# louislung/DAE_RNN_News_Recommendation

Measured on NVIDIA H100. Metric: articles/sec, higher is better.
Workload: dtype f32

## Files before the change

dae_rnn_news_recommendation_b200/csrc/gemm_tc.cu:

```cuda
#include <cuda.h>
#include <cuda_bf16.h>
#include <type_traits>
#include "common.cuh"

namespace dae {

constexpr int BLOCK_M = 128;
constexpr int BLOCK_K = 64;
constexpr int WGMMA_K = 16;
constexpr int kThreads = 384;
constexpr int kDecodeN = 128;

__device__ __forceinline__ uint32_t smem_u32(const void* p) { return (uint32_t)__cvta_generic_to_shared(p); }

__device__ __forceinline__ void mbar_init(uint64_t* bar, uint32_t count) {
  asm volatile("mbarrier.init.shared::cta.b64 [%0], %1;" ::"r"(smem_u32(bar)), "r"(count));
}
__device__ __forceinline__ void mbar_expect_tx(uint64_t* bar, uint32_t bytes) {
  asm volatile("mbarrier.arrive.expect_tx.shared::cta.b64 _, [%0], %1;" ::"r"(smem_u32(bar)), "r"(bytes) : "memory");
}
__device__ __forceinline__ void mbar_arrive(uint64_t* bar) {
  asm volatile("mbarrier.arrive.shared::cta.b64 _, [%0];" ::"r"(smem_u32(bar)) : "memory");
}
__device__ __forceinline__ bool mbar_try_wait(uint64_t* bar, uint32_t parity) {
// ... 79 lines not shown
  d |= (uint64_t)layout << 62;
  return d;
}


template <int TA, int TB>
__device__ __forceinline__ void wgmma_n128(float (&d)[64], uint64_t da, uint64_t db, uint32_t scale_d) {
  asm volatile(
      "{\n"
      ".reg .pred p;\n"
      "setp.ne.b32 p, %66, 0;\n"
      "wgmma.mma_async.sync.aligned.m64n128k16.f32.bf16.bf16 "
      "{%0, %1, %2, %3, %4, %5, %6, %7, %8, %9, %10, %11, %12, %13, %14, %15, %16, %17, %18, %19, %20, %21, %22, %23, %24, %25, %26, %27, %28, %29, %30, %31, %32, %33, %34, %35, %36, %37, %38, %39, %40, %41, %42, %43, %44, %45, %46, %47, %48, %49, %50, %51, %52, %53, %54, %55, %56, %57, %58, %59, %60, %61, %62, %63}, %64, %65, p, 1, 1, %67, %68;\n"
      "}\n"
      : "+f"(d[0]), "+f"(d[1]), "+f"(d[2]), "+f"(d[3]), "+f"(d[4]), "+f"(d[5]), "+f"(d[6]), "+f"(d[7]), "+f"(d[8]), "+f"(d[9]), "+f"(d[10]), "+f"(d[11]), "+f"(d[12]), "+f"(d[13]), "+f"(d[14]), "+f"(d[15]), "+f"(d[16]), "+f"(d[17]), "+f"(d[18]), "+f"(d[19]), "+f"(d[20]), "+f"(d[21]), "+f"(d[22]), "+f"(d[23]), "+f"(d[24]), "+f"(d[25]), "+f"(d[26]), "+f"(d[27]), "+f"(d[28]), "+f"(d[29]), "+f"(d[30]), "+f"(d[31]), "+f"(d[32]), "+f"(d[33]), "+f"(d[34]), "+f"(d[35]), "+f"(d[36]), "+f"(d[37]), "+f"(d[38]), "+f"(d[39]), "+f"(d[40]), "+f"(d[41]), "+f"(d[42]), "+f"(d[43]), "+f"(d[44]), "+f"(d[45]), "+f"(d[46]), "+f"(d[47]), "+f"(d[48]), "+f"(d[49]), "+f"(d[50]), "+f"(d[51]), "+f"(d[52]), "+f"(d[53]), "+f"(d[54]), "+f"(d[55]), "+f"(d[56]), "+f"(d[57]), "+f"(d[58]), "+f"(d[59]), "+f"(d[60]), "+f"(d[61]), "+f"(d[62]), "+f"(d[63])
      : "l"(da), "l"(db), "r"(scale_d), "n"(TA), "n"(TB));
}

template <int TA, int TB>
__device__ __forceinline__ void wgmma_n64(float (&d)[32], uint64_t da, uint64_t db, uint32_t scale_d) {
  asm volatile(
      "{\n"
      ".reg .pred p;\n"
      "setp.ne.b32 p, %34, 0;\n"
      "wgmma.mma_async.sync.aligned.m64n64k16.f32.bf16.bf16 "
      "{%0, %1, %2, %3, %4, %5, %6, %7, %8, %9, %10, %11, %12, %13, %14, %15, %16, %17, %18, %19, %20, %21, %22, %23, %24, %25, %26, %27, %28, %29, %30, %31}, %32, %33, p, 1, 1, %35, %36;\n"
      "}\n"
      : "+f"(d[0]), "+f"(d[1]), "+f"(d[2]), "+f"(d[3]), "+f"(d[4]), "+f"(d[5]), "+f"(d[6]), "+f"(d[7]), "+f"(d[8]), "+f"(d[9]), "+f"(d[10]), "+f"(d[11]), "+f"(d[12]), "+f"(d[13]), "+f"(d[14]), "+f"(d[15]), "+f"(d[16]), "+f"(d[17]), "+f"(d[18]), "+f"(d[19]), "+f"(d[20]), "+f"(d[21]), "+f"(d[22]), "+f"(d[23]), "+f"(d[24]), "+f"(d[25]), "+f"(d[26]), "+f"(d[27]), "+f"(d[28]), "+f"(d[29]), "+f"(d[30]), "+f"(d[31])
      : "l"(da), "l"(db), "r"(scale_d), "n"(TA), "n"(TB));
}
// ... 7 lines not shown
  int a_sym_kb;
  float alpha;
  float* C;
  int64_t ldc;
  int n_store;
  int special_col;
  float* special_out;
  const int64_t* indptr; const int32_t* indices; const float* values; const int32_t* rows;
  const float* bv; const float* weight; const double* stats;
  __nv_bfloat16* dz_hi; __nv_bfloat16* dz_lo; int64_t ld_dz;
  float* row_loss_part;
  const int32_t* tile_ptr;
};

struct Sched {
  int tiles_m, tiles, kb_total, kb_per_split, n_work, stream, w, n_cta;
  long long u, u_end;
  __device__ __forceinline__ void init(const GemmParams& p, int block_n, int pair = 0, int block_k = BLOCK_K) {
    const int cta = pair ? (int)(blockIdx.x >> 1) : (int)blockIdx.x;
    n_cta = pair ? (int)(gridDim.x >> 1) : (int)gridDim.x;
    tiles_m = (p.M + BLOCK_M - 1) / BLOCK_M;
    if (pair) tiles_m = (tiles_m + 1) / 2;
    tiles = tiles_m * ((p.N + block_n - 1) / block_n);
    kb_total = (p.K + block_k - 1) / block_k;
    stream = p.stream_k;
    kb_per_split = (kb_total + p.k_splits - 1) / p.k_splits;
    n_work = tiles * p.k_splits;
    w = cta;
    const long long U = (long long)tiles * kb_total;
    u = (long long)cta * U / n_cta;
    u_end = (long long)(cta + 1) * U / n_cta;
  }
  __device__ __forceinline__ bool next(int& mb, int& nb, int& kb0, int& kb1) {
    int tile;
    if (stream) {
      if (u >= u_end) return false;
      tile = (int)(u / kb_total);
      kb0 = (int)(u - (long long)tile * kb_total);
      const long long left = u_end - u;
      kb1 = (left < (long long)(kb_total - kb0)) ? kb0 + (int)left : kb_total;
      u += kb1 - kb0;
    } else {
      if (w >= n_work) return false;
      tile = w % tiles;
      kb0 = (w / tiles) * kb_per_split;
      kb1 = min(kb_total, kb0 + kb_per_split);
      w += n_cta;
    }
    mb = tile % tiles_m;
    nb = tile / tiles_m;
    return true;
  }
};

__device__ __forceinline__ uint32_t pack_bf16(float a, float b) {
  const __nv_bfloat162 v = __floats2bfloat162_rn(a, b);
  return *reinterpret_cast<const uint32_t*>(&v);
}
__device__ __forceinline__ float f_rcp(float x) { float r; asm("rcp.approx.ftz.f32 %0, %1;" : "=f"(r) : "f"(x)); return r; }
__device__ __forceinline__ float f_lg2(float x) { float r; asm("lg2.approx.ftz.f32 %0, %1;" : "=f"(r) : "f"(x)); return r; }
__device__ __forceinline__ float f_ex2(float x) { float r; asm("ex2.approx.ftz.f32 %0, %1;" : "=f"(r) : "f"(x)); return r; }
constexpr float kLog2e = 1.4426950408889634f;

template <int ACT>
__device__ __forceinline__ float act_fast(float z) {
// ... 54 lines not shown
    }
    const float p01 = a[0] * a[1], p23 = a[2] * a[3], P = p01 * p23;
    ok = ok && (P <= 22026.0f);
    const float Rs = f_rcp(P) * sc;
    lsum += f_lg2(P);
    const float r23 = Rs * p23, r01 = Rs * p01;
    const float dz0 = t[0] * (r23 * a[1]), dz1 = t[1] * (r23 * a[0]), dz2 = t[2] * (r01 * a[3]), dz3 = t[3] * (r01 * a[2]);
    const uint32_t h0 = pack_bf16(dz0, dz1), h1 = pack_bf16(dz2, dz3);
    hpk[2 * g] = h0; hpk[2 * g + 1] = h1;
    lpk[2 * g] = pack_bf16(dz0 - __uint_as_float(h0 << 16), dz1 - __uint_as_float(h0 & 0xffff0000u));
    lpk[2 * g + 1] = pack_bf16(dz2 - __uint_as_float(h1 << 16), dz3 - __uint_as_float(h1 & 0xffff0000u));
  }
  return ok;
}

template <int BLOCK_N, int TA, int TB, int BK = BLOCK_K>
__device__ __forceinline__ void mma_kblock(float (&acc)[BLOCK_N / 2], uint32_t sa_hi, uint32_t sa_lo, uint32_t sb_hi, uint32_t sb_lo,
                                           bool first) {
  static_assert(BK == 64 || (BK == 32 && !TA && !TB), "32-wide k-blocks are K-major only");
  constexpr uint32_t layout = BK == 64 ? 1u : 2u, sbo = BK == 64 ? 1024u : 512u;
  constexpr uint32_t a_lbo = TA ? 8192u : 16u, b_lbo = TB ? 8192u : 16u;
  constexpr uint32_t a_step = TA ? 2048u : 32u, b_step = TB ? 2048u : 32u;
#pragma unroll
  for (int k = 0; k < BK / WGMMA_K; ++k) {
    const uint64_t da_hi = make_desc(sa_hi + k * a_step, a_lbo, sbo, layout), da_lo = make_desc(sa_lo + k * a_step, a_lbo, sbo, layout);
    const uint64_t db_hi = make_desc(sb_hi + k * b_step, b_lbo, sbo, layout), db_lo = make_desc(sb_lo + k * b_step, b_lbo, sbo, layout);
    const uint32_t sc = (first && k == 0) ? 0u : 1u;
    if constexpr (BLOCK_N == 128) {
      wgmma_n128<TA, TB>(acc, da_lo, db_hi, sc);
      wgmma_n128<TA, TB>(acc, da_hi, db_lo, 1u);
      wgmma_n128<TA, TB>(acc, da_hi, db_hi, 1u);
    } else {
      wgmma_n64<TA, TB>(acc, da_lo, db_hi, sc);
      wgmma_n64<TA, TB>(acc, da_hi, db_lo, 1u);
      wgmma_n64<TA, TB>(acc, da_hi, db_hi, 1u);
    }
  }
}

__device__ __forceinline__ void stage_ld16(const float* src, uint32_t (&r)[16]) {
#pragma unroll
  for (int q = 0; q < 4; ++q) {
    const float4 v = reinterpret_cast<const float4*>(src)[q];
// ... 50 lines not shown
      } else if (!p.b_mn) {
        tma_load_2d(tm_b_hi, &full_bar[stage], sb_hi, kbb * BK, nb * BLOCK_N);
        tma_load_2d(tm_b_lo, &full_bar[stage], sb_lo, kbb * BK, nb * BLOCK_N);
      } else {
#pragma unroll
        for (int j = 0; j < BLOCK_N / 64; ++j) {
          tma_load_2d(tm_b_hi, &full_bar[stage], sb_hi + j * (64 * BK * 2), nb * BLOCK_N + j * 64, kbb * BK);
          tma_load_2d(tm_b_lo, &full_bar[stage], sb_lo + j * (64 * BK * 2), nb * BLOCK_N + j * 64, kbb * BK);
        }
      }
      if (++stage == STAGES) { stage = 0; phase ^= 1; }
    }
  }
}

template <int BLOCK_N, int STAGES, int PAIR, int MAJ, int BK = BLOCK_K>
__device__ __forceinline__ void mma_work_item(float (&acc)[BLOCK_N / 2], const GemmParams& p, uint8_t* smem, uint64_t* full_bar,
                                              uint64_t* empty_bar, int wg, int lane, uint32_t crank, int& stage, uint32_t& phase,
                                              int kb0, int kb1) {
  constexpr int A_TILE = BLOCK_M * BK * 2;
  constexpr int B_TILE = BLOCK_N * BK * 2;
  constexpr int STAGE_BYTES = 2 * A_TILE + 2 * B_TILE;
  auto release = [&](int s) {
    __syncwarp();
    if (lane == 0) { mbar_arrive(&empty_bar[s]); if (PAIR) mbar_arrive_cluster(&empty_bar[s], crank ^ 1u); }
  };
  int prev = -1;
  auto run_k = [&](auto ta, auto tb, int kb_begin, int kb_end) {
    for (int kb = kb_begin; kb < kb_end; ++kb) {
      mbar_wait(&full_bar[stage], phase);
      const uint32_t sa_hi = smem_u32(smem + stage * STAGE_BYTES) + wg * (64 * BK * 2);
      const uint32_t sa_lo = sa_hi + A_TILE;
      const uint32_t sb_hi = smem_u32(smem + stage * STAGE_BYTES) + 2 * A_TILE, sb_lo = sb_hi + B_TILE;
      wgmma_fence();
      mma_kblock<BLOCK_N, decltype(ta)::value, decltype(tb)::value, BK>(acc, sa_hi, sa_lo, sb_hi, sb_lo, kb == kb0);
      wgmma_commit();
      wgmma_wait<1>();
      if (prev >= 0) release(prev);
      prev = stage;
      if (++stage == STAGES) { stage = 0; phase ^= 1; }
    }
  };
  using K0 = std::integral_constant<int, 0>;
  using K1 = std::integral_constant<int, 1>;
  if constexpr ((MAJ & 4) != 0) {
    run_k(K0{}, K1{}, kb0, min(kb1, p.a_sym_kb));
    run_k(K1{}, K1{}, max(kb0, p.a_sym_kb), kb1);
  } else {
    run_k(std::integral_constant<int, MAJ & 1>{}, std::integral_constant<int, (MAJ >> 1) & 1>{}, kb0, kb1);
  }
// ... 95 lines not shown
                float* dst = p.C + (int64_t)mm * p.ldc + n;
                if (p.atomic) atomicAdd(dst, v); else *dst = v;
              }
            }
          }
        }
      }
    }
  }

  if (PAIR) cluster_sync_all();
}

constexpr int kDecodeThreads = 640;
constexpr int kDecodeBK = 32;
constexpr int kDecodeStages = 4;
constexpr int kRegsProducer = 32, kRegsMma = 104, kRegsEpilogue = 120;
static_assert(128 * kRegsProducer + 256 * kRegsMma + 256 * kRegsEpilogue <= kDecodeThreads * 96, "register budget");

template <int R> __device__ __forceinline__ void regs_dec() { asm volatile("setmaxnreg.dec.sync.aligned.u32 %0;" ::"n"(R)); }
template <int R> __device__ __forceinline__ void regs_inc() { asm volatile("setmaxnreg.inc.sync.aligned.u32 %0;" ::"n"(R)); }

template <int ACT, int LOSS>
__global__ void __launch_bounds__(kDecodeThreads, 1) decode_fused_kernel(const __grid_constant__ CUtensorMap tm_a_hi,
                                                                         const __grid_constant__ CUtensorMap tm_a_lo,
                                                                         const __grid_constant__ CUtensorMap tm_b_hi,
                                                                         const __grid_constant__ CUtensorMap tm_b_lo,
                                                                         const GemmParams p) {
  constexpr int BLOCK_N = kDecodeN, STAGES = kDecodeStages, BK = kDecodeBK;
  constexpr int STAGE_BYTES = 2 * BLOCK_M * BK * 2 + 2 * BLOCK_N * BK * 2;
  constexpr int SROW = BLOCK_N + 4;
  constexpr int kParts = 2;
  constexpr int HALF_N = BLOCK_N / kParts;
  constexpr bool kFast = (ACT == DAE_ACT_SIGMOID) && (LOSS == DAE_LOSS_CE);
  extern __shared__ __align__(1024) uint8_t smem_raw[];
  uint8_t* smem = reinterpret_cast<uint8_t*>((reinterpret_cast<uintptr_t>(smem_raw) + 1023) & ~(uintptr_t)1023);
  float* stg = reinterpret_cast<float*>(smem + STAGES * STAGE_BYTES);
  __shared__ __align__(8) uint64_t full_bar[STAGES], empty_bar[STAGES], staged_bar[2], drained_bar[2];
  __shared__ float s_bias[2][BLOCK_N];
  __shared__ float s_biasc[kFast ? 2 : 1][kFast ? BLOCK_N : 1];
  __shared__ __align__(16) uint8_t s_stage[8][2][32][48];

  const int warp = threadIdx.x >> 5, lane = threadIdx.x & 31;
  const int role = warp >> 2;
  Sched sched;

  if (warp == 0 && lane == 0) { prefetch_tmap(&tm_a_hi); prefetch_tmap(&tm_a_lo); prefetch_tmap(&tm_b_hi); prefetch_tmap(&tm_b_lo); }
  if (warp == 1 && lane == 0) {
    for (int s = 0; s < STAGES; ++s) { mbar_init(&full_bar[s], 1); mbar_init(&empty_bar[s], 8); }
    for (int h = 0; h < 2; ++h) { mbar_init(&staged_bar[h], 4); mbar_init(&drained_bar[h], 4); }
    fence_barrier_init();
  }
  __syncthreads();

  if (role == 0) {
    regs_dec<kRegsProducer>();
    sched.init(p, BLOCK_N, 0, BK);
    if (warp == 0 && lane == 0)
      tma_produce<BLOCK_N, STAGES, 0, BK>(p, sched, smem, full_bar, empty_bar, 0u, &tm_a_hi, &tm_a_lo, &tm_b_hi, &tm_b_lo, &tm_a_hi, &tm_a_lo);
  } else if (role <= 2) {
    regs_inc<kRegsMma>();
    sched.init(p, BLOCK_N, 0, BK);
    const int h = role - 1;
    const int wi = warp & 3;
    float acc[BLOCK_N / 2];
#pragma unroll
    for (int i = 0; i < BLOCK_N / 2; ++i) acc[i] = 0.0f;
    int stage = 0; uint32_t phase = 0, tphase = 0;
    int mb, nb, kb0, kb1;
    while (sched.next(mb, nb, kb0, kb1)) {
      mma_work_item<BLOCK_N, STAGES, 0, 0, BK>(acc, p, smem, full_bar, empty_bar, h, lane, 0u, stage, phase, kb0, kb1);
      mbar_wait(&drained_bar[h], tphase ^ 1);
      const int r0 = h * 64 + wi * 16 + (lane >> 2), c0 = 2 * (lane & 3);
#pragma unroll
      for (int j = 0; j < BLOCK_N / 8; ++j) {
        *reinterpret_cast<float2*>(&stg[r0 * SROW + 8 * j + c0]) = make_float2(acc[4 * j], acc[4 * j + 1]);
        *reinterpret_cast<float2*>(&stg[(r0 + 8) * SROW + 8 * j + c0]) = make_float2(acc[4 * j + 2], acc[4 * j + 3]);
      }
      __syncwarp();
      if (lane == 0) mbar_arrive(&staged_bar[h]);
      tphase ^= 1;
    }
  } else {
    regs_inc<kRegsEpilogue>();
    sched.init(p, BLOCK_N, 0, BK);
    const int h = role - 3;
    const int ew = warp - 12;
    const int wi = warp & 3;
    const int quarter = h * 2 + (wi & 1);
    const int half = wi >> 1;
    const int row_in_tile = quarter * 32 + lane;
    const int tid = threadIdx.x - 128 * role;
    const int tiles_n = (p.N + BLOCK_N - 1) / BLOCK_N;
    uint8_t* stg_hi = reinterpret_cast<uint8_t*>(&s_stage[ew][0][0][0]);
    uint8_t* stg_lo = reinterpret_cast<uint8_t*>(&s_stage[ew][1][0][0]);
    const int rsub = lane >> 1, csub = lane & 1;
    uint32_t tphase = 0;
    int mb, nb, kb0, kb1;
    while (sched.next(mb, nb, kb0, kb1)) {
      const float* srow = stg + row_in_tile * SROW + half * HALF_N;
      const int m = mb * BLOCK_M + row_in_tile;
      const int n0 = nb * BLOCK_N + half * HALF_N;
      int64_t pc = 0, pe = 0;
      int c0 = 0x7fffffff, c1 = 0x7fffffff, c2 = 0x7fffffff;
      float v0 = 0.0f, v1 = 0.0f, v2 = 0.0f;
      float sc = 0.0f;
      if (m < p.M) {
        const int64_t row = p.rows ? (int64_t)p.rows[m] : (int64_t)m;
        const int64_t rbeg = p.indptr[row];
        const int32_t* tp = p.tile_ptr + (int64_t)m * (kParts * tiles_n + 1) + nb * kParts + half;
        pc = rbeg + tp[0]; pe = rbeg + tp[1];
        if (pc < pe) { c0 = p.indices[pc]; v0 = p.values[pc]; }
        if (pc + 1 < pe) { c1 = p.indices[pc + 1]; v1 = p.values[pc + 1]; }
        if (pc + 2 < pe) { c2 = p.indices[pc + 2]; v2 = p.values[pc + 2]; }
        sc = (p.weight ? p.weight[m] : 1.0f) / ((float)p.stats[DAE_STAT_SUM_W] + kEps);
      }
      named_bar_sync(1 + h, 128);
      {
        const float b = (nb * BLOCK_N + tid < p.N) ? p.bv[nb * BLOCK_N + tid] : 0.0f;
        s_bias[h][tid] = b;
        if (kFast) s_biasc[h][tid] = b * kLog2e;
      }
      mbar_wait(&staged_bar[h], tphase);
      named_bar_sync(1 + h, 128);
      const float inv_sc = (sc != 0.0f) ? 1.0f / sc : 0.0f;
      const bool edge = (n0 + HALF_N > p.N);
      float lsum = 0.0f;
      const int m_base = mb * BLOCK_M + quarter * 32;
      const int n_lim = edge ? p.N : 0x7fffffff;
#pragma unroll 1
      for (int c = 0; c < HALF_N / 16; ++c) {
        uint32_t r[16];
        stage_ld16(srow + c * 16, r);
        const int nc = n0 + c * 16;
        if (m < p.M) {
          const float* bias = &s_bias[h][half * HALF_N + c * 16];
          uint32_t hpk[8], lpk[8];
          bool fast_ok = false;
          if (kFast && !edge) {
            const float l0 = lsum;
            fast_ok = decode_chunk_sigmoid_ce(r, &s_biasc[h][half * HALF_N + c * 16], sc, hpk, lpk, lsum);
            if (!fast_ok) { lsum = l0; decode_chunk_generic<ACT, LOSS>(r, bias, sc, edge, n_lim, nc, hpk, lpk, lsum); }
          } else {
            decode_chunk_generic<ACT, LOSS>(r, bias, sc, edge, n_lim, nc, hpk, lpk, lsum);
          }
          uint4* sh = reinterpret_cast<uint4*>(stg_hi + lane * 48);
          uint4* sl = reinterpret_cast<uint4*>(stg_lo + lane * 48);
          sh[0] = make_uint4(hpk[0], hpk[1], hpk[2], hpk[3]); sh[1] = make_uint4(hpk[4], hpk[5], hpk[6], hpk[7]);
          sl[0] = make_uint4(lpk[0], lpk[1], lpk[2], lpk[3]); sl[1] = make_uint4(lpk[4], lpk[5], lpk[6], lpk[7]);
          while (c0 < nc + 16) {
            const float x = v0;
            const int j = c0 - nc;
            __nv_bfloat16* ph = reinterpret_cast<__nv_bfloat16*>(stg_hi + lane * 48) + j;
            __nv_bfloat16* pl = reinterpret_cast<__nv_bfloat16*>(stg_lo + lane * 48) + j;
            float d;
            if (kFast && fast_ok && sc != 0.0f) d = (__bfloat162float(*ph) + __bfloat162float(*pl)) * inv_sc;
            else d = act_fast<ACT>(select16(r, j) + bias[j]);
            const float gp = act_grad_from_y<ACT>(d);
            float dz;
            if (LOSS == DAE_LOSS_CE) {
              const float a = d + kEps, b = (1.0f - d) + kEps;
              const float la = f_lg2(a), lb = f_lg2(b);
              lsum += lb - (x * la + (1.0f - x) * lb);
              dz = sc * gp * ((1.0f - x) * f_rcp(b) - x * f_rcp(a));
            } else {
              const float e2 = x - d;
              lsum += e2 * e2 - d * d;
              dz = -2.0f * sc * e2 * gp;
            }
            const __nv_bfloat16 hb = __float2bfloat16_rn(dz);
            *ph = hb;
            *pl = __float2bfloat16_rn(dz - __bfloat162float(hb));
            ++pc;
            c0 = c1; v0 = v1; c1 = c2; v1 = v2;
            c2 = 0x7fffffff;
            if (pc + 2 < pe) { c2 = p.indices[pc + 2]; v2 = p.values[pc + 2]; }
          }
        }
        __syncwarp();
        if (nc < p.ld_dz) {
#pragma unroll
          for (int i = 0; i < 2; ++i) {
            const int rr = rsub + 16 * i;
            if (m_base + rr < p.M) {
              const int64_t off = (int64_t)(m_base + rr) * p.ld_dz + nc + csub * 8;
              *reinterpret_cast<uint4*>(p.dz_hi + off) = *reinterpret_cast<const uint4*>(stg_hi + rr * 48 + csub * 16);
              *reinterpret_cast<uint4*>(p.dz_lo + off) = *reinterpret_cast<const uint4*>(stg_lo + rr * 48 + csub * 16);
            }
          }
        }
        __syncwarp();
      }
      if (lane == 0) mbar_arrive(&drained_bar[h]);
      tphase ^= 1;
      if (m < p.M) atomicAdd(p.row_loss_part + m, (LOSS == DAE_LOSS_CE) ? lsum * 0.6931471805599453f : lsum);
    }
  }
}

constexpr int kTopkMaxK = 32;
constexpr int kTopkMaxSplits = 32;
constexpr int kTopkMinTiles = 4;
constexpr int kTopkBK = 64;
constexpr int kTopkStages = 2;

struct TopkParams {
  GemmParams g;
  int k, splits;
  int exclude;
  int64_t diag_offset;
// ... 350 lines not shown
    at[0].val.clusterDim.x = 2; at[0].val.clusterDim.y = 1; at[0].val.clusterDim.z = 1;
    cfg.attrs = at; cfg.numAttrs = 1;
    DAE_CUDA(cudaLaunchKernelEx(&cfg, kern, ta_hi, ta_lo, tb_hi, tb_lo, tat_hi, tat_lo, p));
  }
  return DAE_OK;
}

template <int BLOCK_N, int STAGES, int PAIR>
static int launch_gemm(const Operand& A, const Operand& B, GemmParams p, cudaStream_t st) {
  if (!A.mn_major && !B.mn_major) return launch_gemm_maj<BLOCK_N, STAGES, PAIR, 0>(A, B, p, st);
  if (A.mn_major && !B.mn_major) return launch_gemm_maj<BLOCK_N, STAGES, PAIR, 1>(A, B, p, st);
  if (!A.mn_major) return launch_gemm_maj<BLOCK_N, STAGES, PAIR, 2>(A, B, p, st);
  return launch_gemm_maj<BLOCK_N, STAGES, PAIR, 3>(A, B, p, st);
}

template <int ACT, int LOSS>
static int launch_decode(const Operand& A, const Operand& B, const GemmParams& p, cudaStream_t st) {
  CUtensorMap ta_hi, ta_lo, tb_hi, tb_lo;
  int rc;
  if ((rc = make_map(&ta_hi, A.hi, p.K, p.M, A.ld, BLOCK_M, kDecodeBK))) return rc;
  if ((rc = make_map(&ta_lo, A.lo, p.K, p.M, A.ld, BLOCK_M, kDecodeBK))) return rc;
  if ((rc = make_map(&tb_hi, B.hi, p.K, p.N, B.ld, kDecodeN, kDecodeBK))) return rc;
  if ((rc = make_map(&tb_lo, B.lo, p.K, p.N, B.ld, kDecodeN, kDecodeBK))) return rc;
  constexpr int smem = kDecodeStages * (2 * BLOCK_M * kDecodeBK * 2 + 2 * kDecodeN * kDecodeBK * 2) + BLOCK_M * (kDecodeN + 4) * 4 + 1024;
  auto kern = decode_fused_kernel<ACT, LOSS>;
  static bool attr_done[64] = {false};
  if ((rc = ensure_smem_attr(kern, smem, attr_done))) return rc;
  const int tiles = ((p.M + BLOCK_M - 1) / BLOCK_M) * ((p.N + kDecodeN - 1) / kDecodeN);
  const int n = tiles < sm_count() ? tiles : sm_count();
  kern<<<n, kDecodeThreads, smem, st>>>(ta_hi, ta_lo, tb_hi, tb_lo, p);
  return DAE_OK;
}

template <int KMAX>
static int launch_topk(const Operand& A, const Operand& B, const TopkParams& tp, cudaStream_t st) {
  CUtensorMap ta_hi, ta_lo, tb_hi, tb_lo;
  int rc;
  const GemmParams& p = tp.g;
  if ((rc = make_map(&ta_hi, A.hi, p.K, p.M, A.ld, BLOCK_M, kTopkBK))) return rc;
  if ((rc = make_map(&ta_lo, A.lo, p.K, p.M, A.ld, BLOCK_M, kTopkBK))) return rc;
  if ((rc = make_map(&tb_hi, B.hi, p.K, p.N, B.ld, kDecodeN, kTopkBK))) return rc;
  if ((rc = make_map(&tb_lo, B.lo, p.K, p.N, B.ld, kDecodeN, kTopkBK))) return rc;
  constexpr int smem = kTopkStages * (2 * BLOCK_M * kTopkBK * 2 + 2 * kDecodeN * kTopkBK * 2) + BLOCK_M * (kDecodeN + 4) * 4 + 1024;
  auto kern = topk_kernel<KMAX>;
  static bool attr_done[64] = {false};
  if ((rc = ensure_smem_attr(kern, smem, attr_done))) return rc;
// ... 126 lines not shown
  DAE_CHECK_LAUNCH("dae_decode_prepare");
  return DAE_OK;
}

extern "C" int dae_decode_fused_bf16x3(int32_t Brows, int32_t F, int32_t K, const void* e_hi, const void* e_lo, int64_t lde,
                                       const void* w_hi, const void* w_lo, int64_t ldw, const int64_t* indptr, const int32_t* indices,
                                       const float* values, const int32_t* rows, const float* bv, int32_t dec_act, int32_t loss_func,
                                       const float* weight, const double* stats, void* dz_hi, void* dz_lo, int64_t ld_dz,
                                       float* row_loss_part, int32_t* tile_ptr, int32_t prepared, void* stream) {
  DAE_REQUIRE(e_hi && e_lo && w_hi && w_lo && indptr && indices && values && bv && stats && dz_hi && dz_lo && row_loss_part && tile_ptr,
              "dae_decode_fused_bf16x3: null pointer");
  DAE_REQUIRE(loss_func == DAE_LOSS_CE || loss_func == DAE_LOSS_MSE, "dae_decode_fused_bf16x3: cosine loss uses the unfused path");
  DAE_REQUIRE(lde % 8 == 0 && ldw % 8 == 0 && ld_dz % 32 == 0 && ld_dz >= F, "dae_decode_fused_bf16x3: bad leading dimensions");
  cudaStream_t st = (cudaStream_t)stream;
  GemmParams p{};
  p.M = Brows; p.N = F; p.K = K; p.k_splits = 1; p.alpha = 1.0f; p.special_col = -1;
  p.indptr = indptr; p.indices = indices; p.values = values; p.rows = rows; p.bv = bv; p.weight = weight; p.stats = stats;
  p.dz_hi = (__nv_bfloat16*)dz_hi; p.dz_lo = (__nv_bfloat16*)dz_lo; p.ld_dz = ld_dz; p.row_loss_part = row_loss_part;
  p.tile_ptr = tile_ptr;
  if (!prepared) {
    int rc0 = dae_decode_prepare(Brows, F, indptr, indices, rows, row_loss_part, tile_ptr, stream);
    if (rc0) return rc0;
  }
  Operand A{e_hi, e_lo, lde, 0}, B{w_hi, w_lo, ldw, 0};
  int rc = 0;
#define DAE_DEC(ACT, LOSS) rc = launch_decode<ACT, LOSS>(A, B, p, st)
  if (loss_func == DAE_LOSS_CE) {
    if (dec_act == DAE_ACT_SIGMOID) DAE_DEC(DAE_ACT_SIGMOID, DAE_LOSS_CE);
    else if (dec_act == DAE_ACT_TANH) DAE_DEC(DAE_ACT_TANH, DAE_LOSS_CE);
    else DAE_DEC(DAE_ACT_NONE, DAE_LOSS_CE);
  } else {
    if (dec_act == DAE_ACT_SIGMOID) DAE_DEC(DAE_ACT_SIGMOID, DAE_LOSS_MSE);
    else if (dec_act == DAE_ACT_TANH) DAE_DEC(DAE_ACT_TANH, DAE_LOSS_MSE);
    else DAE_DEC(DAE_ACT_NONE, DAE_LOSS_MSE);
  }
#undef DAE_DEC
  if (rc) return rc;
  DAE_CHECK_LAUNCH("dae_decode_fused_bf16x3");
  return DAE_OK;
}

// ... 37 lines not shown
```

Baseline: 2.051 million.

## Swap fused decode GEMM operands so features tile M and batch tiles N

The fused decode kernel now treats the decoder weight (features) as the M operand and the embeddings (batch rows) as the N operand, with an n-fast tile order so consecutive CTAs share weight tiles. It adds an m64n136 wgmma variant and picks a 136- or 128-row batch tile at launch, based on which gives fewer wave-quantised rows. The epilogue is reorganised to stage transposed accumulators and write dz in place in the staging buffer, with a fifth chunk for the extra 8 rows. The aim is better wave balance and reuse of weight tiles, at the cost of strided transposed shared-memory stores and more accumulator registers in the MMA warps.

```diff
diff --git a/dae_rnn_news_recommendation_b200/csrc/gemm_tc.cu b/dae_rnn_news_recommendation_b200/csrc/gemm_tc.cu
--- a/dae_rnn_news_recommendation_b200/csrc/gemm_tc.cu
+++ b/dae_rnn_news_recommendation_b200/csrc/gemm_tc.cu
@@ -117,6 +117,19 @@
       "{%0, %1, %2, %3, %4, %5, %6, %7, %8, %9, %10, %11, %12, %13, %14, %15, %16, %17, %18, %19, %20, %21, %22, %23, %24, %25, %26, %27, %28, %29, %30, %31, %32, %33, %34, %35, %36, %37, %38, %39, %40, %41, %42, %43, %44, %45, %46, %47, %48, %49, %50, %51, %52, %53, %54, %55, %56, %57, %58, %59, %60, %61, %62, %63}, %64, %65, p, 1, 1, %67, %68;\n"
       "}\n"
       : "+f"(d[0]), "+f"(d[1]), "+f"(d[2]), "+f"(d[3]), "+f"(d[4]), "+f"(d[5]), "+f"(d[6]), "+f"(d[7]), "+f"(d[8]), "+f"(d[9]), "+f"(d[10]), "+f"(d[11]), "+f"(d[12]), "+f"(d[13]), "+f"(d[14]), "+f"(d[15]), "+f"(d[16]), "+f"(d[17]), "+f"(d[18]), "+f"(d[19]), "+f"(d[20]), "+f"(d[21]), "+f"(d[22]), "+f"(d[23]), "+f"(d[24]), "+f"(d[25]), "+f"(d[26]), "+f"(d[27]), "+f"(d[28]), "+f"(d[29]), "+f"(d[30]), "+f"(d[31]), "+f"(d[32]), "+f"(d[33]), "+f"(d[34]), "+f"(d[35]), "+f"(d[36]), "+f"(d[37]), "+f"(d[38]), "+f"(d[39]), "+f"(d[40]), "+f"(d[41]), "+f"(d[42]), "+f"(d[43]), "+f"(d[44]), "+f"(d[45]), "+f"(d[46]), "+f"(d[47]), "+f"(d[48]), "+f"(d[49]), "+f"(d[50]), "+f"(d[51]), "+f"(d[52]), "+f"(d[53]), "+f"(d[54]), "+f"(d[55]), "+f"(d[56]), "+f"(d[57]), "+f"(d[58]), "+f"(d[59]), "+f"(d[60]), "+f"(d[61]), "+f"(d[62]), "+f"(d[63])
+      : "l"(da), "l"(db), "r"(scale_d), "n"(TA), "n"(TB));
+}
+
+template <int TA, int TB>
+__device__ __forceinline__ void wgmma_n136(float (&d)[68], uint64_t da, uint64_t db, uint32_t scale_d) {
+  asm volatile(
+      "{\n"
+      ".reg .pred p;\n"
+      "setp.ne.b32 p, %70, 0;\n"
+      "wgmma.mma_async.sync.aligned.m64n136k16.f32.bf16.bf16 "
+      "{%0, %1, %2, %3, %4, %5, %6, %7, %8, %9, %10, %11, %12, %13, %14, %15, %16, %17, %18, %19, %20, %21, %22, %23, %24, %25, %26, %27, %28, %29, %30, %31, %32, %33, %34, %35, %36, %37, %38, %39, %40, %41, %42, %43, %44, %45, %46, %47, %48, %49, %50, %51, %52, %53, %54, %55, %56, %57, %58, %59, %60, %61, %62, %63, %64, %65, %66, %67}, %68, %69, p, 1, 1, %71, %72;\n"
+      "}\n"
+      : "+f"(d[0]), "+f"(d[1]), "+f"(d[2]), "+f"(d[3]), "+f"(d[4]), "+f"(d[5]), "+f"(d[6]), "+f"(d[7]), "+f"(d[8]), "+f"(d[9]), "+f"(d[10]), "+f"(d[11]), "+f"(d[12]), "+f"(d[13]), "+f"(d[14]), "+f"(d[15]), "+f"(d[16]), "+f"(d[17]), "+f"(d[18]), "+f"(d[19]), "+f"(d[20]), "+f"(d[21]), "+f"(d[22]), "+f"(d[23]), "+f"(d[24]), "+f"(d[25]), "+f"(d[26]), "+f"(d[27]), "+f"(d[28]), "+f"(d[29]), "+f"(d[30]), "+f"(d[31]), "+f"(d[32]), "+f"(d[33]), "+f"(d[34]), "+f"(d[35]), "+f"(d[36]), "+f"(d[37]), "+f"(d[38]), "+f"(d[39]), "+f"(d[40]), "+f"(d[41]), "+f"(d[42]), "+f"(d[43]), "+f"(d[44]), "+f"(d[45]), "+f"(d[46]), "+f"(d[47]), "+f"(d[48]), "+f"(d[49]), "+f"(d[50]), "+f"(d[51]), "+f"(d[52]), "+f"(d[53]), "+f"(d[54]), "+f"(d[55]), "+f"(d[56]), "+f"(d[57]), "+f"(d[58]), "+f"(d[59]), "+f"(d[60]), "+f"(d[61]), "+f"(d[62]), "+f"(d[63]), "+f"(d[64]), "+f"(d[65]), "+f"(d[66]), "+f"(d[67])
       : "l"(da), "l"(db), "r"(scale_d), "n"(TA), "n"(TB));
 }
 
@@ -154,14 +167,17 @@
 };
 
 struct Sched {
-  int tiles_m, tiles, kb_total, kb_per_split, n_work, stream, w, n_cta;
+  int tiles_m, tiles_n, tiles, kb_total, kb_per_split, n_work, stream, w, n_cta;
+  bool n_fast;
   long long u, u_end;
-  __device__ __forceinline__ void init(const GemmParams& p, int block_n, int pair = 0, int block_k = BLOCK_K) {
+  __device__ __forceinline__ void init(const GemmParams& p, int block_n, int pair = 0, int block_k = BLOCK_K, bool n_fast_ = false) {
+    n_fast = n_fast_;
     const int cta = pair ? (int)(blockIdx.x >> 1) : (int)blockIdx.x;
     n_cta = pair ? (int)(gridDim.x >> 1) : (int)gridDim.x;
     tiles_m = (p.M + BLOCK_M - 1) / BLOCK_M;
     if (pair) tiles_m = (tiles_m + 1) / 2;
-    tiles = tiles_m * ((p.N + block_n - 1) / block_n);
+    tiles_n = (p.N + block_n - 1) / block_n;
+    tiles = tiles_m * tiles_n;
     kb_total = (p.K + block_k - 1) / block_k;
     stream = p.stream_k;
     kb_per_split = (kb_total + p.k_splits - 1) / p.k_splits;
@@ -187,8 +203,8 @@
       kb1 = min(kb_total, kb0 + kb_per_split);
       w += n_cta;
     }
-    mb = tile % tiles_m;
-    nb = tile / tiles_m;
+    if (n_fast) { nb = tile % tiles_n; mb = tile / tiles_n; }
+    else { mb = tile % tiles_m; nb = tile / tiles_m; }
     return true;
   }
 };
@@ -273,10 +289,11 @@
   return ok;
 }
 
-template <int BLOCK_N, int TA, int TB, int BK = BLOCK_K>
+template <int BLOCK_N, int TA, int TB, int BK = BLOCK_K, bool SWAP = false>
 __device__ __forceinline__ void mma_kblock(float (&acc)[BLOCK_N / 2], uint32_t sa_hi, uint32_t sa_lo, uint32_t sb_hi, uint32_t sb_lo,
                                            bool first) {
   static_assert(BK == 64 || (BK == 32 && !TA && !TB), "32-wide k-blocks are K-major only");
+  static_assert(!SWAP || BLOCK_N == 128 || BLOCK_N == 136, "SWAP is the fused decode's order");
   constexpr uint32_t layout = BK == 64 ? 1u : 2u, sbo = BK == 64 ? 1024u : 512u;
   constexpr uint32_t a_lbo = TA ? 8192u : 16u, b_lbo = TB ? 8192u : 16u;
   constexpr uint32_t a_step = TA ? 2048u : 32u, b_step = TB ? 2048u : 32u;
@@ -285,7 +302,15 @@
     const uint64_t da_hi = make_desc(sa_hi + k * a_step, a_lbo, sbo, layout), da_lo = make_desc(sa_lo + k * a_step, a_lbo, sbo, layout);
     const uint64_t db_hi = make_desc(sb_hi + k * b_step, b_lbo, sbo, layout), db_lo = make_desc(sb_lo + k * b_step, b_lbo, sbo, layout);
     const uint32_t sc = (first && k == 0) ? 0u : 1u;
-    if constexpr (BLOCK_N == 128) {
+    if constexpr (SWAP && BLOCK_N == 136) {
+      wgmma_n136<TA, TB>(acc, da_hi, db_lo, sc);
+      wgmma_n136<TA, TB>(acc, da_lo, db_hi, 1u);
+      wgmma_n136<TA, TB>(acc, da_hi, db_hi, 1u);
+    } else if constexpr (SWAP) {
+      wgmma_n128<TA, TB>(acc, da_hi, db_lo, sc);
+      wgmma_n128<TA, TB>(acc, da_lo, db_hi, 1u);
+      wgmma_n128<TA, TB>(acc, da_hi, db_hi, 1u);
+    } else if constexpr (BLOCK_N == 128) {
       wgmma_n128<TA, TB>(acc, da_lo, db_hi, sc);
       wgmma_n128<TA, TB>(acc, da_hi, db_lo, 1u);
       wgmma_n128<TA, TB>(acc, da_hi, db_hi, 1u);
@@ -366,7 +391,7 @@
   }
 }
 
-template <int BLOCK_N, int STAGES, int PAIR, int MAJ, int BK = BLOCK_K>
+template <int BLOCK_N, int STAGES, int PAIR, int MAJ, int BK = BLOCK_K, bool SWAP = false>
 __device__ __forceinline__ void mma_work_item(float (&acc)[BLOCK_N / 2], const GemmParams& p, uint8_t* smem, uint64_t* full_bar,
                                               uint64_t* empty_bar, int wg, int lane, uint32_t crank, int& stage, uint32_t& phase,
                                               int kb0, int kb1) {
@@ -385,7 +410,7 @@
       const uint32_t sa_lo = sa_hi + A_TILE;
       const uint32_t sb_hi = smem_u32(smem + stage * STAGE_BYTES) + 2 * A_TILE, sb_lo = sb_hi + B_TILE;
       wgmma_fence();
-      mma_kblock<BLOCK_N, decltype(ta)::value, decltype(tb)::value, BK>(acc, sa_hi, sa_lo, sb_hi, sb_lo, kb == kb0);
+      mma_kblock<BLOCK_N, decltype(ta)::value, decltype(tb)::value, BK, SWAP>(acc, sa_hi, sa_lo, sb_hi, sb_lo, kb == kb0);
       wgmma_commit();
       wgmma_wait<1>();
       if (prev >= 0) release(prev);
@@ -511,38 +536,72 @@
 
 constexpr int kDecodeThreads = 640;
 constexpr int kDecodeBK = 32;
-constexpr int kDecodeStages = 4;
+template <int BN> constexpr int decode_stages() { return 4; }
+template <int BN> constexpr int decode_smem() {
+  return decode_stages<BN>() * (2 * BLOCK_M * kDecodeBK * 2 + 2 * BN * kDecodeBK * 2) + BN * (kDecodeN + 4) * 4 + 1024;
+}
 constexpr int kRegsProducer = 32, kRegsMma = 104, kRegsEpilogue = 120;
 static_assert(128 * kRegsProducer + 256 * kRegsMma + 256 * kRegsEpilogue <= kDecodeThreads * 96, "register budget");
 
 template <int R> __device__ __forceinline__ void regs_dec() { asm volatile("setmaxnreg.dec.sync.aligned.u32 %0;" ::"n"(R)); }
 template <int R> __device__ __forceinline__ void regs_inc() { asm volatile("setmaxnreg.inc.sync.aligned.u32 %0;" ::"n"(R)); }
 
-template <int ACT, int LOSS>
-__global__ void __launch_bounds__(kDecodeThreads, 1) decode_fused_kernel(const __grid_constant__ CUtensorMap tm_a_hi,
-                                                                         const __grid_constant__ CUtensorMap tm_a_lo,
-                                                                         const __grid_constant__ CUtensorMap tm_b_hi,
-                                                                         const __grid_constant__ CUtensorMap tm_b_lo,
+struct DecodeCursor {
+  int64_t pc, pe;
+  int c0, c1, c2;
+  float v0, v1, v2;
+  float sc;
+  __device__ __forceinline__ void load(const GemmParams& p, int m, int n_rows, int tiles_f, int ft, int half, int from) {
+    pc = pe = 0;
+    c0 = c1 = c2 = 0x7fffffff;
+    v0 = v1 = v2 = 0.0f;
+    sc = 0.0f;
+    if (m >= n_rows) return;
+    const int64_t row = p.rows ? (int64_t)p.rows[m] : (int64_t)m;
+    const int64_t rbeg = p.indptr[row];
+    const int32_t* tp = p.tile_ptr + (int64_t)m * (2 * tiles_f + 1) + 2 * ft + half;
+    pc = rbeg + tp[0]; pe = rbeg + tp[1];
+    if (pc < pe) { c0 = p.indices[pc]; v0 = p.values[pc]; }
+    if (pc + 1 < pe) { c1 = p.indices[pc + 1]; v1 = p.values[pc + 1]; }
+    if (pc + 2 < pe) { c2 = p.indices[pc + 2]; v2 = p.values[pc + 2]; }
+    sc = (p.weight ? p.weight[m] : 1.0f) / ((float)p.stats[DAE_STAT_SUM_W] + kEps);
+    while (c0 < from) advance(p);
+  }
+  __device__ __forceinline__ void advance(const GemmParams& p) {
+    ++pc;
+    c0 = c1; v0 = v1; c1 = c2; v1 = v2;
+    c2 = 0x7fffffff;
+    if (pc + 2 < pe) { c2 = p.indices[pc + 2]; v2 = p.values[pc + 2]; }
+  }
+};
+
+template <int ACT, int LOSS, int BN>
+__global__ void __launch_bounds__(kDecodeThreads, 1) decode_fused_kernel(const __grid_constant__ CUtensorMap tm_w_hi,
+                                                                         const __grid_constant__ CUtensorMap tm_w_lo,
+                                                                         const __grid_constant__ CUtensorMap tm_e_hi,
+                                                                         const __grid_constant__ CUtensorMap tm_e_lo,
                                                                          const GemmParams p) {
-  constexpr int BLOCK_N = kDecodeN, STAGES = kDecodeStages, BK = kDecodeBK;
-  constexpr int STAGE_BYTES = 2 * BLOCK_M * BK * 2 + 2 * BLOCK_N * BK * 2;
-  constexpr int SROW = BLOCK_N + 4;
-  constexpr int kParts = 2;
-  constexpr int HALF_N = BLOCK_N / kParts;
+  static_assert(BN == 128 || BN == 136, "batch tile of 128 or 136 rows");
+  static_assert(BLOCK_M == kDecodeN, "the feature tile is dae_decode_prepare's column tile");
+  constexpr int STAGES = decode_stages<BN>(), BK = kDecodeBK;
+  constexpr int STAGE_BYTES = 2 * BLOCK_M * BK * 2 + 2 * BN * BK * 2;
+  constexpr int SROW = kDecodeN + 4;
+  constexpr int HALF_F = kDecodeN / 2;
+  constexpr int kChunks = BN > 128 ? 5 : 4;
   constexpr bool kFast = (ACT == DAE_ACT_SIGMOID) && (LOSS == DAE_LOSS_CE);
   extern __shared__ __align__(1024) uint8_t smem_raw[];
   uint8_t* smem = reinterpret_cast<uint8_t*>((reinterpret_cast<uintptr_t>(smem_raw) + 1023) & ~(uintptr_t)1023);
   float* stg = reinterpret_cast<float*>(smem + STAGES * STAGE_BYTES);
   __shared__ __align__(8) uint64_t full_bar[STAGES], empty_bar[STAGES], staged_bar[2], drained_bar[2];
-  __shared__ float s_bias[2][BLOCK_N];
-  __shared__ float s_biasc[kFast ? 2 : 1][kFast ? BLOCK_N : 1];
-  __shared__ __align__(16) uint8_t s_stage[8][2][32][48];
+  __shared__ float s_bias[2][HALF_F];
+  __shared__ float s_biasc[kFast ? 2 : 1][kFast ? HALF_F : 1];
 
   const int warp = threadIdx.x >> 5, lane = threadIdx.x & 31;
   const int role = warp >> 2;
+  const int F = p.M, n_rows = p.N;
   Sched sched;
 
-  if (warp == 0 && lane == 0) { prefetch_tmap(&tm_a_hi); prefetch_tmap(&tm_a_lo); prefetch_tmap(&tm_b_hi); prefetch_tmap(&tm_b_lo); }
+  if (warp == 0 && lane == 0) { prefetch_tmap(&tm_w_hi); prefetch_tmap(&tm_w_lo); prefetch_tmap(&tm_e_hi); prefetch_tmap(&tm_e_lo); }
   if (warp == 1 && lane == 0) {
     for (int s = 0; s < STAGES; ++s) { mbar_init(&full_bar[s], 1); mbar_init(&empty_bar[s], 8); }
     for (int h = 0; h < 2; ++h) { mbar_init(&staged_bar[h], 4); mbar_init(&drained_bar[h], 4); }
@@ -552,27 +611,27 @@
 
   if (role == 0) {
     regs_dec<kRegsProducer>();
-    sched.init(p, BLOCK_N, 0, BK);
+    sched.init(p, BN, 0, BK, true);
     if (warp == 0 && lane == 0)
-      tma_produce<BLOCK_N, STAGES, 0, BK>(p, sched, smem, full_bar, empty_bar, 0u, &tm_a_hi, &tm_a_lo, &tm_b_hi, &tm_b_lo, &tm_a_hi, &tm_a_lo);
+      tma_produce<BN, STAGES, 0, BK>(p, sched, smem, full_bar, empty_bar, 0u, &tm_w_hi, &tm_w_lo, &tm_e_hi, &tm_e_lo, &tm_w_hi, &tm_w_lo);
   } else if (role <= 2) {
     regs_inc<kRegsMma>();
-    sched.init(p, BLOCK_N, 0, BK);
+    sched.init(p, BN, 0, BK, true);
     const int h = role - 1;
     const int wi = warp & 3;
-    float acc[BLOCK_N / 2];
-#pragma unroll
-    for (int i = 0; i < BLOCK_N / 2; ++i) acc[i] = 0.0f;
+    float acc[BN / 2];
+#pragma unroll
+    for (int i = 0; i < BN / 2; ++i) acc[i] = 0.0f;
     int stage = 0; uint32_t phase = 0, tphase = 0;
     int mb, nb, kb0, kb1;
     while (sched.next(mb, nb, kb0, kb1)) {
-      mma_work_item<BLOCK_N, STAGES, 0, 0, BK>(acc, p, smem, full_bar, empty_bar, h, lane, 0u, stage, phase, kb0, kb1);
+      mma_work_item<BN, STAGES, 0, 0, BK, true>(acc, p, smem, full_bar, empty_bar, h, lane, 0u, stage, phase, kb0, kb1);
       mbar_wait(&drained_bar[h], tphase ^ 1);
-      const int r0 = h * 64 + wi * 16 + (lane >> 2), c0 = 2 * (lane & 3);
-#pragma unroll
-      for (int j = 0; j < BLOCK_N / 8; ++j) {
-        *reinterpret_cast<float2*>(&stg[r0 * SROW + 8 * j + c0]) = make_float2(acc[4 * j], acc[4 * j + 1]);
-        *reinterpret_cast<float2*>(&stg[(r0 + 8) * SROW + 8 * j + c0]) = make_float2(acc[4 * j + 2], acc[4 * j + 3]);
+      const int f0 = h * HALF_F + wi * 16 + (lane >> 2), b0 = 2 * (lane & 3);
+#pragma unroll
+      for (int j = 0; j < BN / 8; ++j) {
+        float* s = stg + (8 * j + b0) * SROW + f0;
+        s[0] = acc[4 * j]; s[SROW] = acc[4 * j + 1]; s[8] = acc[4 * j + 2]; s[SROW + 8] = acc[4 * j + 3];
       }
       __syncwarp();
       if (lane == 0) mbar_arrive(&staged_bar[h]);
@@ -580,76 +639,72 @@
     }
   } else {
     regs_inc<kRegsEpilogue>();
-    sched.init(p, BLOCK_N, 0, BK);
+    sched.init(p, BN, 0, BK, true);
     const int h = role - 3;
-    const int ew = warp - 12;
     const int wi = warp & 3;
-    const int quarter = h * 2 + (wi & 1);
-    const int half = wi >> 1;
-    const int row_in_tile = quarter * 32 + lane;
     const int tid = threadIdx.x - 128 * role;
-    const int tiles_n = (p.N + BLOCK_N - 1) / BLOCK_N;
-    uint8_t* stg_hi = reinterpret_cast<uint8_t*>(&s_stage[ew][0][0][0]);
-    uint8_t* stg_lo = reinterpret_cast<uint8_t*>(&s_stage[ew][1][0][0]);
+    const int tiles_f = (F + kDecodeN - 1) / kDecodeN;
     const int rsub = lane >> 1, csub = lane & 1;
     uint32_t tphase = 0;
     int mb, nb, kb0, kb1;
     while (sched.next(mb, nb, kb0, kb1)) {
-      const float* srow = stg + row_in_tile * SROW + half * HALF_N;
-      const int m = mb * BLOCK_M + row_in_tile;
-      const int n0 = nb * BLOCK_N + half * HALF_N;
-      int64_t pc = 0, pe = 0;
-      int c0 = 0x7fffffff, c1 = 0x7fffffff, c2 = 0x7fffffff;
-      float v0 = 0.0f, v1 = 0.0f, v2 = 0.0f;
-      float sc = 0.0f;
-      if (m < p.M) {
-        const int64_t row = p.rows ? (int64_t)p.rows[m] : (int64_t)m;
-        const int64_t rbeg = p.indptr[row];
-        const int32_t* tp = p.tile_ptr + (int64_t)m * (kParts * tiles_n + 1) + nb * kParts + half;
-        pc = rbeg + tp[0]; pe = rbeg + tp[1];
-        if (pc < pe) { c0 = p.indices[pc]; v0 = p.values[pc]; }
-        if (pc + 1 < pe) { c1 = p.indices[pc + 1]; v1 = p.values[pc + 1]; }
-        if (pc + 2 < pe) { c2 = p.indices[pc + 2]; v2 = p.values[pc + 2]; }
-        sc = (p.weight ? p.weight[m] : 1.0f) / ((float)p.stats[DAE_STAT_SUM_W] + kEps);
-      }
+      const int n0 = mb * kDecodeN + h * HALF_F;
+      const int row0 = nb * BN;
+      const int m_end = min(n_rows, row0 + BN);
+      DecodeCursor cur, nxt;
+      cur.load(p, row0 + tid, m_end, tiles_f, mb, h, n0);
+      if (kChunks > 4) nxt.load(p, row0 + 128 + lane, m_end, tiles_f, mb, h, n0 + 16 * wi);
       named_bar_sync(1 + h, 128);
-      {
-        const float b = (nb * BLOCK_N + tid < p.N) ? p.bv[nb * BLOCK_N + tid] : 0.0f;
+      if (tid < HALF_F) {
+        const float b = (n0 + tid < F) ? p.bv[n0 + tid] : 0.0f;
         s_bias[h][tid] = b;
         if (kFast) s_biasc[h][tid] = b * kLog2e;
       }
       mbar_wait(&staged_bar[h], tphase);
       named_bar_sync(1 + h, 128);
-      const float inv_sc = (sc != 0.0f) ? 1.0f / sc : 0.0f;
-      const bool edge = (n0 + HALF_N > p.N);
+      const bool edge = (n0 + HALF_F > F);
+      const int n_lim = edge ? F : 0x7fffffff;
+      int r_in = tid;
+      int m_base = row0 + 32 * wi;
+      float inv_sc = (cur.sc != 0.0f) ? 1.0f / cur.sc : 0.0f;
       float lsum = 0.0f;
-      const int m_base = mb * BLOCK_M + quarter * 32;
-      const int n_lim = edge ? p.N : 0x7fffffff;
 #pragma unroll 1
-      for (int c = 0; c < HALF_N / 16; ++c) {
-        uint32_t r[16];
-        stage_ld16(srow + c * 16, r);
+      for (int i = 0; i < kChunks; ++i) {
+        int c = i;
+        if (i == 4) {
+          if (row0 + r_in < m_end) atomicAdd(p.row_loss_part + row0 + r_in, (LOSS == DAE_LOSS_CE) ? lsum * 0.6931471805599453f : lsum);
+          lsum = 0.0f;
+          cur = nxt;
+          inv_sc = (cur.sc != 0.0f) ? 1.0f / cur.sc : 0.0f;
+          r_in = 128 + lane; m_base = row0 + 128; c = wi;
+        }
+        const int m = row0 + r_in;
+        const float sc = cur.sc;
         const int nc = n0 + c * 16;
-        if (m < p.M) {
-          const float* bias = &s_bias[h][half * HALF_N + c * 16];
+        uint8_t* cbase = reinterpret_cast<uint8_t*>(stg + h * HALF_F + c * 16);
+        uint8_t* mine = cbase + r_in * (SROW * 4);
+        if (m < m_end) {
+          uint32_t r[16];
+          stage_ld16(reinterpret_cast<const float*>(mine), r);
+          const float* bias = &s_bias[h][c * 16];
           uint32_t hpk[8], lpk[8];
           bool fast_ok = false;
           if (kFast && !edge) {
             const float l0 = lsum;
-            fast_ok = decode_chunk_sigmoid_ce(r, &s_biasc[h][half * HALF_N + c * 16], sc, hpk, lpk, lsum);
+            fast_ok = decode_chunk_sigmoid_ce(r, &s_biasc[h][c * 16], sc, hpk, lpk, lsum);
             if (!fast_ok) { lsum = l0; decode_chunk_generic<ACT, LOSS>(r, bias, sc, edge, n_lim, nc, hpk, lpk, lsum); }
           } else {
             decode_chunk_generic<ACT, LOSS>(r, bias, sc, edge, n_lim, nc, hpk, lpk, lsum);
           }
-          uint4* sh = reinterpret_cast<uint4*>(stg_hi + lane * 48);
-          uint4* sl = reinterpret_cast<uint4*>(stg_lo + lane * 48);
+          uint4* sh = reinterpret_cast<uint4*>(mine);
+          uint4* sl = reinterpret_cast<uint4*>(mine + 32);
           sh[0] = make_uint4(hpk[0], hpk[1], hpk[2], hpk[3]); sh[1] = make_uint4(hpk[4], hpk[5], hpk[6], hpk[7]);
           sl[0] = make_uint4(lpk[0], lpk[1], lpk[2], lpk[3]); sl[1] = make_uint4(lpk[4], lpk[5], lpk[6], lpk[7]);
-          while (c0 < nc + 16) {
-            const float x = v0;
-            const int j = c0 - nc;
-            __nv_bfloat16* ph = reinterpret_cast<__nv_bfloat16*>(stg_hi + lane * 48) + j;
-            __nv_bfloat16* pl = reinterpret_cast<__nv_bfloat16*>(stg_lo + lane * 48) + j;
+          while (cur.c0 < nc + 16) {
+            const float x = cur.v0;
+            const int j = cur.c0 - nc;
+            __nv_bfloat16* ph = reinterpret_cast<__nv_bfloat16*>(mine) + j;
+            __nv_bfloat16* pl = reinterpret_cast<__nv_bfloat16*>(mine + 32) + j;
             float d;
             if (kFast && fast_ok && sc != 0.0f) d = (__bfloat162float(*ph) + __bfloat162float(*pl)) * inv_sc;
             else d = act_fast<ACT>(select16(r, j) + bias[j]);
@@ -668,21 +723,19 @@
             const __nv_bfloat16 hb = __float2bfloat16_rn(dz);
             *ph = hb;
             *pl = __float2bfloat16_rn(dz - __bfloat162float(hb));
-            ++pc;
-            c0 = c1; v0 = v1; c1 = c2; v1 = v2;
-            c2 = 0x7fffffff;
-            if (pc + 2 < pe) { c2 = p.indices[pc + 2]; v2 = p.values[pc + 2]; }
+            cur.advance(p);
           }
         }
         __syncwarp();
         if (nc < p.ld_dz) {
 #pragma unroll
-          for (int i = 0; i < 2; ++i) {
-            const int rr = rsub + 16 * i;
-            if (m_base + rr < p.M) {
+          for (int i2 = 0; i2 < 2; ++i2) {
+            const int rr = rsub + 16 * i2;
+            if (m_base + rr < m_end) {
               const int64_t off = (int64_t)(m_base + rr) * p.ld_dz + nc + csub * 8;
-              *reinterpret_cast<uint4*>(p.dz_hi + off) = *reinterpret_cast<const uint4*>(stg_hi + rr * 48 + csub * 16);
-              *reinterpret_cast<uint4*>(p.dz_lo + off) = *reinterpret_cast<const uint4*>(stg_lo + rr * 48 + csub * 16);
+              const uint8_t* src = cbase + (m_base - row0 + rr) * (SROW * 4) + csub * 16;
+              *reinterpret_cast<uint4*>(p.dz_hi + off) = *reinterpret_cast<const uint4*>(src);
+              *reinterpret_cast<uint4*>(p.dz_lo + off) = *reinterpret_cast<const uint4*>(src + 32);
             }
           }
         }
@@ -690,7 +743,7 @@
       }
       if (lane == 0) mbar_arrive(&drained_bar[h]);
       tphase ^= 1;
-      if (m < p.M) atomicAdd(p.row_loss_part + m, (LOSS == DAE_LOSS_CE) ? lsum * 0.6931471805599453f : lsum);
+      if (row0 + r_in < m_end) atomicAdd(p.row_loss_part + row0 + r_in, (LOSS == DAE_LOSS_CE) ? lsum * 0.6931471805599453f : lsum);
     }
   }
 }
@@ -1071,22 +1124,34 @@
   return launch_gemm_maj<BLOCK_N, STAGES, PAIR, 3>(A, B, p, st);
 }
 
-template <int ACT, int LOSS>
-static int launch_decode(const Operand& A, const Operand& B, const GemmParams& p, cudaStream_t st) {
-  CUtensorMap ta_hi, ta_lo, tb_hi, tb_lo;
+template <int ACT, int LOSS, int BN>
+static int launch_decode(const Operand& W, const Operand& E, const GemmParams& p, cudaStream_t st) {
+  CUtensorMap tw_hi, tw_lo, te_hi, te_lo;
   int rc;
-  if ((rc = make_map(&ta_hi, A.hi, p.K, p.M, A.ld, BLOCK_M, kDecodeBK))) return rc;
-  if ((rc = make_map(&ta_lo, A.lo, p.K, p.M, A.ld, BLOCK_M, kDecodeBK))) return rc;
-  if ((rc = make_map(&tb_hi, B.hi, p.K, p.N, B.ld, kDecodeN, kDecodeBK))) return rc;
-  if ((rc = make_map(&tb_lo, B.lo, p.K, p.N, B.ld, kDecodeN, kDecodeBK))) return rc;
-  constexpr int smem = kDecodeStages * (2 * BLOCK_M * kDecodeBK * 2 + 2 * kDecodeN * kDecodeBK * 2) + BLOCK_M * (kDecodeN + 4) * 4 + 1024;
-  auto kern = decode_fused_kernel<ACT, LOSS>;
+  if ((rc = make_map(&tw_hi, W.hi, p.K, p.M, W.ld, BLOCK_M, kDecodeBK))) return rc;
+  if ((rc = make_map(&tw_lo, W.lo, p.K, p.M, W.ld, BLOCK_M, kDecodeBK))) return rc;
+  if ((rc = make_map(&te_hi, E.hi, p.K, p.N, E.ld, BN, kDecodeBK))) return rc;
+  if ((rc = make_map(&te_lo, E.lo, p.K, p.N, E.ld, BN, kDecodeBK))) return rc;
+  constexpr int smem = decode_smem<BN>();
+  auto kern = decode_fused_kernel<ACT, LOSS, BN>;
   static bool attr_done[64] = {false};
   if ((rc = ensure_smem_attr(kern, smem, attr_done))) return rc;
-  const int tiles = ((p.M + BLOCK_M - 1) / BLOCK_M) * ((p.N + kDecodeN - 1) / kDecodeN);
+  const int tiles = ((p.M + BLOCK_M - 1) / BLOCK_M) * ((p.N + BN - 1) / BN);
   const int n = tiles < sm_count() ? tiles : sm_count();
-  kern<<<n, kDecodeThreads, smem, st>>>(ta_hi, ta_lo, tb_hi, tb_lo, p);
+  kern<<<n, kDecodeThreads, smem, st>>>(tw_hi, tw_lo, te_hi, te_lo, p);
   return DAE_OK;
+}
+
+static int decode_batch_tile(int F, int B) {
+  const long long tiles_f = (F + kDecodeN - 1) / kDecodeN, sms = sm_count();
+  const long long cost128 = (tiles_f * ((B + 127) / 128) + sms - 1) / sms * 128;
+  const long long cost136 = (tiles_f * ((B + 135) / 136) + sms - 1) / sms * 136;
+  return cost136 < cost128 ? 136 : 128;
+}
+
+template <int ACT, int LOSS>
+static int launch_decode_any(const Operand& W, const Operand& E, const GemmParams& p, cudaStream_t st) {
+  return decode_batch_tile(p.M, p.N) == 136 ? launch_decode<ACT, LOSS, 136>(W, E, p, st) : launch_decode<ACT, LOSS, 128>(W, E, p, st);
 }
 
 template <int KMAX>
@@ -1243,7 +1308,7 @@
   DAE_REQUIRE(lde % 8 == 0 && ldw % 8 == 0 && ld_dz % 32 == 0 && ld_dz >= F, "dae_decode_fused_bf16x3: bad leading dimensions");
   cudaStream_t st = (cudaStream_t)stream;
   GemmParams p{};
-  p.M = Brows; p.N = F; p.K = K; p.k_splits = 1; p.alpha = 1.0f; p.special_col = -1;
+  p.M = F; p.N = Brows; p.K = K; p.k_splits = 1; p.alpha = 1.0f; p.special_col = -1;
   p.indptr = indptr; p.indices = indices; p.values = values; p.rows = rows; p.bv = bv; p.weight = weight; p.stats = stats;
   p.dz_hi = (__nv_bfloat16*)dz_hi; p.dz_lo = (__nv_bfloat16*)dz_lo; p.ld_dz = ld_dz; p.row_loss_part = row_loss_part;
   p.tile_ptr = tile_ptr;
@@ -1251,9 +1316,9 @@
     int rc0 = dae_decode_prepare(Brows, F, indptr, indices, rows, row_loss_part, tile_ptr, stream);
     if (rc0) return rc0;
   }
-  Operand A{e_hi, e_lo, lde, 0}, B{w_hi, w_lo, ldw, 0};
+  Operand Wop{w_hi, w_lo, ldw, 0}, Eop{e_hi, e_lo, lde, 0};
   int rc = 0;
-#define DAE_DEC(ACT, LOSS) rc = launch_decode<ACT, LOSS>(A, B, p, st)
+#define DAE_DEC(ACT, LOSS) rc = launch_decode_any<ACT, LOSS>(Wop, Eop, p, st)
   if (loss_func == DAE_LOSS_CE) {
     if (dec_act == DAE_ACT_SIGMOID) DAE_DEC(DAE_ACT_SIGMOID, DAE_LOSS_CE);
     else if (dec_act == DAE_ACT_TANH) DAE_DEC(DAE_ACT_TANH, DAE_LOSS_CE);
```

Result: no change. 2.065 million, median of 6 (+0.7%).
